# joybio/multiPrime

Measured on AMD Instinct MI355X. Metric: candidate x sequence coverage evals/s, higher is better.
Workload: dtype u32; 1 GPU; synthetic MSA 1048576 x 1000, k=18, v=1, 8 candidates/window, 950 windows, strict -c 2,3,-1 per GPU x 1 GPU(s) = BASELINE configs[3] itself (SURVEY 8d input 4; synthetic 1M x 1 kb; shape 1x1: row shards x window groups); rows_per_gpu=1048576, rows_total=1048576, cols=1000, k=18, variation=1, candidates_per_window=8, windows=950, parallelism=one GPU holds every row

## Files before the change

multiprime_amd/csrc/common.hpp:

```cpp
#pragma once

#include "../../include/mprime.h"

#include <hip/hip_runtime.h>

#include <algorithm>
#include <cstdarg>
#include <cstdio>
#include <cstdlib>
#include <cstring>
#include <numeric>
#include <utility>
#include <chrono>
#include <mutex>
#include <unordered_map>
#include <vector>

namespace mp {

constexpr int kBlock = 256;
constexpr uint32_t kEmpty = 0xFFFFFFFFu;
constexpr int kHashSlots = 4096;
constexpr int kHashLimit = 3584;
constexpr int kEvalCC = 8;
// ... 107 lines not shown
    hipStream_t ex_stream = nullptr;
    int ex_pending = 0;
    std::mutex ex_mu;
    int32_t *extra_off = nullptr;
    uint32_t *extra_words = nullptr;
    int n_extra = 0;
    std::vector<int32_t> h_patch_off, h_extra_off;
    uint32_t *pplanes = nullptr, *pvalid = nullptr;
    uint32_t *qplanes = nullptr, *qvalid = nullptr;
    bool qp_dirty = true;
    mp::PatchWin *pwin = nullptr;
    size_t pp_words = 0, pv_words = 0;
    int max_npw = 0;
    bool pp_dirty = true;
    unsigned long long *g_key = nullptr;
    uint32_t *g_cnt = nullptr, *g_min = nullptr;
    uint32_t *g_gap = nullptr;
    int32_t *g_idx = nullptr;
    int g_slots = 0;
    long long u_cap = 0, u_n = 0;
    uint32_t *u_b0 = nullptr, *u_b1 = nullptr, *u_g = nullptr;
    int32_t *u_count = nullptr, *u_first = nullptr, *labels = nullptr, *u_over = nullptr, *u_wcount = nullptr;
    int64_t *u_wbase = nullptr;
    unsigned long long *u_total = nullptr;
    std::vector<int64_t> h_wbase;
    std::vector<int32_t> h_wcount;
    double gate_threshold = 0;
    std::vector<uint8_t> h_wskip;
    uint8_t *dm_loss = nullptr;
    double *dm_dg = nullptr;
    std::vector<uint8_t> dm_loss_host;
    std::vector<double> dm_dg_host;
    unsigned long long *mask_f = nullptr, *mask_r = nullptr;
    size_t mask_words = 0;
    int n_masks = 0;
    int n_cand = 0, n_items = 0, n_padded = 0;
    mp::EvalItem *items = nullptr;
    uint4 *cand_n = nullptr;
    uint32_t *cand_symT = nullptr, *cand_diff = nullptr, *chain_events = nullptr;
    mp::ChainItem *chain_items = nullptr;
    void *x_items = nullptr;
    uint32_t *x_events = nullptr;
    int32_t *x_cand_out = nullptr;
    int x_n = 0, x_n_events = 0;
    int32_t *table_ids = nullptr;
    int n_chain = 0, n_table = 0, n_events = 0, max_steps = 0;
    std::vector<mp::ChainItem> h_chains;
    std::vector<uint32_t> h_events;
    std::vector<int32_t> h_cand_out;
    uint32_t *chain_prog = nullptr;
    size_t chain_prog_n = 0;
    mp::EvalForm form;
    mp::SlideBand *slide_bands = nullptr;
    uint32_t *slide_iters = nullptr, *slide_recs = nullptr;
    size_t slide_n_iters = 0;
    int slide_items = 0, slide_n_bands = 0, slide_max_items = 0, slide_ns = 0, slide_gw = 0;
    uint32_t slide_spos = 0, slide_fmask = 0, slide_rmask = 0, slide_fpos = 0, slide_rpos = 0;
    bool slide_fast = false;
    mp::ChainItem *chain_rest = nullptr;
    mp::ChainItem *chain_slid = nullptr;
    int n_rest = 0, rest_max_steps = 0;
    unsigned launch_seq = 0;
    int32_t *cand_out = nullptr;
    uint64_t sF = 0, sR = 0;
    unsigned long long *tmp_out = nullptr;
    int tmp_out_n = 0;
    struct PoolBlock { void *p; size_t bytes; hipEvent_t released; };
    std::vector<hipEvent_t> pool_events;
    std::unordered_map<void *, size_t> pool_live;
    std::vector<PoolBlock> pool;
    size_t pool_bytes = 0;
    long long pool_hits = 0, pool_misses = 0;
    int pool_on = -1;
    std::mutex pool_mu;
    unsigned long long *stats_buf = nullptr;
    size_t stats_buf_n = 0;
    std::vector<std::pair<hipEvent_t, hipEvent_t>> ev_busy, ev_free;
    double ev_ms = 0;
    std::vector<float> ev_samples, ev_last;
    int ev_n = 0;
    uint8_t *h_stage = nullptr;
    size_t h_stage_bytes = 0;
    bool h_stage_pinned = false;
    uint8_t *h_stats = nullptr;
    size_t h_stats_bytes = 0, stats_pending_f = 0, stats_pending_t = 0;
    bool h_stats_pinned = false;
    hipEvent_t stats_ev = nullptr;
    uint8_t *h_ring = nullptr;
    bool h_ring_pinned = false;
    hipEvent_t h_ring_ev[3] = {nullptr, nullptr, nullptr};
    uint8_t *sq_bytes = nullptr;
    int64_t *sq_roff = nullptr;
    unsigned long long *sq_code = nullptr, *sq_flag = nullptr;
    int64_t *sq_woff = nullptr;
    int32_t sq_n = 0;
    size_t sq_total = 0, sq_words = 0;
    std::vector<int64_t> sq_roff_host;
    int32_t *ot_out = nullptr;
    int64_t ot_n = 0;
    std::vector<uint8_t> ot_key;
    double ot_ms[4] = {0, 0, 0, 0};
    int64_t ot_counts[7] = {0, 0, 0, 0, 0, 0, 0};
    uint8_t *an_code = nullptr;
    uint32_t *an_kmer = nullptr;
    int32_t *an_table = nullptr;
    int32_t *an_col = nullptr, *an_colinv = nullptr;
    int32_t an_n = 0, an_L = 0, an_slots = 0;
// ... 122 lines not shown
```

multiprime_amd/csrc/evalslide.hip:

```cpp
#include "common.hpp"
#include "bitslice.hpp"
#include "slidecore.hpp"
#include "evalslide.hpp"
#include "chainbody.hpp"

using namespace mp;

namespace {

typedef unsigned int u32x4 __attribute__((ext_vector_type(4)));
typedef unsigned int u32x2 __attribute__((ext_vector_type(2)));

struct SlideKernArgs {
    SlideArgs A;
    const uint32_t *cols32;
    const uint32_t *excl32;
    int nw32;
    unsigned long long *out;
    int wc, wc_pad;
    int max_items;
    int n_slide_blocks;
    EvalChainArgs chain;
    unsigned long long *clear;
    uint32_t n_clear;
    int patch_words;
    unsigned long long *stamps;
};

template <int GW>
struct DevEnv {
    const SlideKernArgs &K;
    __amdgpu_buffer_rsrc_t rs_cols, rs_excl;
    int voff, lane;
    uint32_t row_bytes;
    bool live;
    uint32_t *ring;
    uint32_t *tab;
    uint32_t itv;
    uint32_t live_mask;

    __device__ __forceinline__ DevEnv(const SlideKernArgs &k) : K(k) {}
    __device__ __forceinline__ void progress(int quarter) const {
#ifndef SLIDE_NO_PRIO
        if (quarter <= 0) __builtin_amdgcn_s_setprio(3);
        else if (quarter == 1) __builtin_amdgcn_s_setprio(2);
        else if (quarter == 2) __builtin_amdgcn_s_setprio(1);
        else __builtin_amdgcn_s_setprio(0);
#endif
    }
    __device__ __forceinline__ void stamp(int i) const {
        if (K.stamps && threadIdx.x == 0) K.stamps[(size_t)blockIdx.x * 8 + i] = wall_clock64();
    }
    __device__ __forceinline__ SlideBand uband(int b) const {
        const SlideBand *p = K.A.bands + b;
        SlideBand r;
        r.w0 = __builtin_amdgcn_readfirstlane(p->w0); r.n_win = __builtin_amdgcn_readfirstlane(p->n_win);
        r.item0 = __builtin_amdgcn_readfirstlane(p->item0); r.n_items = __builtin_amdgcn_readfirstlane(p->n_items);
        r.iter0 = __builtin_amdgcn_readfirstlane(p->iter0); r.pad = 0;
        return r;
    }
    __device__ __forceinline__ void load_iters(int idx) { itv = K.A.iters[(size_t)idx + (size_t)lane]; }
    __device__ __forceinline__ uint32_t iter_word(int j) const { return (uint32_t)__builtin_amdgcn_readlane((int)itv, j); }
    typedef const uint32_t __attribute__((address_space(4))) * ConstWords;
    struct Rec { uint32_t w[8], sm_lo, sm_hi, flags; ConstWords p; };
    __device__ __forceinline__ Rec load_rec(int item) const {
        Rec r;
        r.p = (ConstWords)(K.A.recs + (size_t)__builtin_amdgcn_readfirstlane(item) * kSlideRec);
#pragma unroll
        for (int q = 0; q < 8; q++) r.w[q] = r.p[q];
        r.sm_lo = r.p[24]; r.sm_hi = r.p[25]; r.flags = r.p[28];
        return r;
    }
    __device__ __forceinline__ uint32_t rec_word(const Rec &r, int q) const {
        return q < 8 ? r.w[q] : (q == 24 ? r.sm_lo : (q == 25 ? r.sm_hi : (q == 28 ? r.flags : r.p[q])));
    }
    __device__ __forceinline__ uint32_t rec_word_dyn(const Rec &r, int q) const { return r.p[q]; }
    template <int AUX = 0>
    __device__ __forceinline__ void load(__amdgpu_buffer_rsrc_t rs, int soff, uint32_t (&d)[GW]) const {
        if constexpr (GW == 4) {
            const u32x4 v = __builtin_amdgcn_raw_buffer_load_b128(rs, voff, soff, AUX);
            d[0] = v.x; d[1] = v.y; d[2] = v.z; d[3] = v.w;
        } else if constexpr (GW == 2) {
            const u32x2 v = __builtin_amdgcn_raw_buffer_load_b64(rs, voff, soff, AUX);
            d[0] = v.x; d[1] = v.y;
        } else {
            d[0] = __builtin_amdgcn_raw_buffer_load_b32(rs, voff, soff, AUX);
        }
    }
#ifndef SLIDE_EXP_ONE_ROW
#define SLIDE_EXP_ONE_ROW 0
#endif
#ifndef SLIDE_COL_AUX
#define SLIDE_COL_AUX 2
#endif
#ifndef SLIDE_EVT_AUX
#define SLIDE_EVT_AUX 0
#endif
    __device__ __forceinline__ void fetch(uint32_t row_off, uint32_t (&d)[GW]) const {
        load<SLIDE_COL_AUX>(rs_cols, SLIDE_EXP_ONE_ROW == 1 || SLIDE_EXP_ONE_ROW == 3 ? 0 : (int)row_off, d);
    }
    __device__ __forceinline__ void fetch_event(uint32_t row_off, uint32_t (&d)[GW]) const {
// ... 46 lines not shown
            "v_add_u32_dpp %8, %8, %8 row_ror:8 row_mask:0xf bank_mask:0x3\n\t"
            "v_add_u32_dpp %0, %2, %2 row_ror:8 row_mask:0xf bank_mask:0xc\n\t"
            "v_add_u32_dpp %4, %6, %6 row_ror:8 row_mask:0xf bank_mask:0xc\n\t"
            "v_add_u32_dpp %8, %10, %10 row_ror:8 row_mask:0xf bank_mask:0xc\n\t"
            "v_add_u32_dpp %0, %0, %0 quad_perm:[1,0,3,2] row_mask:0xf bank_mask:0xf\n\t"
            "v_add_u32_dpp %4, %4, %4 quad_perm:[1,0,3,2] row_mask:0xf bank_mask:0xf\n\t"
            "v_add_u32_dpp %8, %8, %8 quad_perm:[1,0,3,2] row_mask:0xf bank_mask:0xf\n\t"
            "v_add_u32_dpp %0, %0, %0 quad_perm:[2,3,0,1] row_mask:0xf bank_mask:0xf\n\t"
            "v_add_u32_dpp %4, %4, %4 quad_perm:[2,3,0,1] row_mask:0xf bank_mask:0xf\n\t"
            "v_add_u32_dpp %8, %8, %8 quad_perm:[2,3,0,1] row_mask:0xf bank_mask:0xf\n\t"
            "s_nop 1"
            : "+v"(x0), "+v"(x1), "+v"(x2), "+v"(x3), "+v"(x4), "+v"(x5), "+v"(x6), "+v"(x7), "+v"(x8), "+v"(x9), "+v"(x10), "+v"(x11));
        typedef unsigned int u32pair __attribute__((ext_vector_type(2)));
        const u32pair s01 = __builtin_amdgcn_permlane16_swap(x0, x4, false, false);
        const uint32_t a = s01.x + s01.y;
        const u32pair s22 = __builtin_amdgcn_permlane16_swap(x8, x8, false, false);
        const uint32_t b = s22.x + s22.y;
        const u32pair h = __builtin_amdgcn_permlane32_swap(a, b, false, false);
        const uint32_t tot = h.x + h.y;
        if (lane < 48 && (lane & 3) == 0) atomicAdd(&tab[idx * 12 + (lane >> 4) * 4 + ((lane >> 2) & 3)], tot);
    }
};

#ifndef SLIDE_MIN_WAVES
#define SLIDE_MIN_WAVES 1
#endif
template <int LV, int GW, bool FAST>
__global__ __launch_bounds__(kBlock, GW == 4 ? 1 : SLIDE_MIN_WAVES) void eval_slide_kernel(const SlideKernArgs K) {
    extern __shared__ __align__(16) uint32_t lds[];
    clear_counters(K.clear, K.n_clear, blockIdx.x, gridDim.x);
    if (K.stamps && threadIdx.x == 0) K.stamps[(size_t)blockIdx.x * 8] = wall_clock64();
    if ((int)blockIdx.x >= K.n_slide_blocks) {
        const unsigned pb = blockIdx.x - (unsigned)K.n_slide_blocks, wv = threadIdx.x >> 6;
#ifndef SLIDE_PATCH_PRIO
#define SLIDE_PATCH_PRIO 3
#endif
        __builtin_amdgcn_s_setprio(SLIDE_PATCH_PRIO);
        if (K.patch_words == 1) {
            const bool negative = (int)pb >= K.chain.patch.n_blocks;
            const unsigned unit = (pb - (negative ? (unsigned)K.chain.patch.n_blocks : 0u)) * (kBlock / 64) + wv;
            eval_patch_wave<LV>(K.chain, lds + wv * 12, lds + 64 + wv * (64 * kPatchEvents), unit, negative);
        } else {
            uint32_t(&s_part)[kBlock / 64][12] = *reinterpret_cast<uint32_t(*)[kBlock / 64][12]>(lds);
            eval_chain_block<LV, 8, 4>(K.chain, s_part, pb);
        }
        if (K.stamps && threadIdx.x == 0) K.stamps[(size_t)blockIdx.x * 8 + 7] = wall_clock64();
        return;
    }
    const int slice = (int)(blockIdx.x % (unsigned)K.wc_pad), band = (int)(blockIdx.x / (unsigned)K.wc_pad);
    if (slice >= K.wc) return;
    const int wv = (int)(threadIdx.x >> 6), lane = (int)(threadIdx.x & 63);
    const int ring_words = K.A.k * 64 * GW;
    uint32_t *tab = lds + (kBlock / 64) * ring_words;
    DevEnv<GW> env(K);
    env.lane = lane;
    env.ring = lds + wv * ring_words + lane * GW;
    env.tab = tab;
    env.itv = 0u;
    const int word0 = (slice * kBlock + (int)threadIdx.x) * GW;
    env.live = word0 < K.nw32;
    env.voff = env.live ? word0 * 4 : 0x7FFFFF00;
    env.live_mask = env.live ? 0xFFFFFFFFu : 0u;
    env.row_bytes = (uint32_t)K.nw32 * 4u;
    env.rs_cols = __builtin_amdgcn_make_buffer_rsrc(const_cast<uint32_t *>(K.cols32), 0, 0x7FFFFF00, 0x00020000);
    env.rs_excl = __builtin_amdgcn_make_buffer_rsrc(const_cast<uint32_t *>(K.excl32), 0, 0x7FFFFF00, 0x00020000);
    const SlideBand bd = env.uband(band);
    for (int i = (int)threadIdx.x; i < bd.n_items * 12; i += kBlock) tab[i] = 0u;
    __syncthreads();
    env.stamp(1);
    const bool wave_live = (slice * kBlock + wv * 64) * GW < K.nw32;
    if (wave_live) slide_band<LV, GW, true, false, FAST>(env, K.A, band);
    env.stamp(4);
    __syncthreads();
    env.stamp(5);
    int live_waves = 0;
    for (int w = 0; w < kBlock / 64; w++) live_waves += (slice * kBlock + w * 64) * GW < K.nw32 ? 1 : 0;
    const uint32_t rows = (uint32_t)live_waves * 64u * 32u * GW;
    const int n_entries = bd.n_items * 24;
    for (int i0 = (int)threadIdx.x; i0 < n_entries; i0 += 4 * kBlock) {
        int oc[4];
        uint32_t map[4];
#pragma unroll
        for (int u = 0; u < 4; u++) {
            const int i = i0 + u * kBlock, ic = i < n_entries ? i : (int)threadIdx.x;
            const uint32_t *rec = K.A.recs + (size_t)(bd.item0 + ic / 24) * kSlideRec;
            oc[u] = (int)rec[8 + (ic % 24) / 3];
            map[u] = rec[26];
        }
#pragma unroll
        for (int u = 0; u < 4; u++) {
            const int i = i0 + u * kBlock;
            if (i >= n_entries || oc[u] < 0) continue;
            const int item = i / 24, r = i % 24, t = r / 3, kind = r % 3;
            const int slot = (int)((map[u] >> (4 * t)) & 15u);
            const uint32_t *row = tab + item * 12;
            const uint32_t out1 = row[slot] & 0xFFFFu, outF = row[slot] >> 16, outR = (row[8 + (slot >> 1)] >> (16 * (slot & 1))) & 0xFFFFu;
            const uint32_t val = kind == 0 ? rows - out1 : out1 - (kind == 1 ? outF : outR);
            if (val) atomicAdd(&K.out[(size_t)oc[u] * 3 + kind], (unsigned long long)val);
        }
    }
    env.stamp(6);
}

typedef void (*SlideFn)(const SlideKernArgs);

}

namespace mp {

void free_slide(mp_ctx *c) {
    dev_free(c, &c->slide_bands, (size_t)c->slide_n_bands);
    dev_free(c, &c->slide_iters, c->slide_n_iters);
    dev_free(c, &c->slide_recs, (size_t)c->slide_items * kSlideRec);
    dev_free(c, &c->chain_rest, (size_t)c->n_rest);
    dev_free(c, &c->chain_slid, (size_t)c->slide_items);
    c->slide_items = c->slide_n_bands = c->slide_max_items = 0;
    c->slide_n_iters = 0;
    c->n_rest = c->rest_max_steps = 0;
}

int upload_eval_slide(mp_ctx *c, const std::vector<ChainItem> &chains, const std::vector<uint32_t> &events, const std::vector<int32_t> &cand_out) {
    free_slide(c);
    const char *se = getenv("MP_EVAL_SLIDE");
    if (chains.empty() || c->v > 3 || c->k <= c->v || (se ? atoi(se) != 1 : c->n_pad <= 262144)) return MP_OK;
    const int nw32 = c->n_pad / 32, n_cols = c->n_chunks * 32;
    if (((unsigned long long)n_cols * 4ull + 1ull) * (unsigned long long)nw32 * 4ull >= 0x7FFFFFFFull) return MP_OK;
    if ((unsigned long long)c->n_win * (unsigned long long)nw32 * 4ull >= 0x7FFFFFFFull) return MP_OK;
    int gw = 2;
    if (const char *e = getenv("MP_SLIDE_GW")) { const int g = atoi(e); if (g == 1 || g == 2 || g == 4) gw = g; }
    const int wc = (nw32 + kBlock * gw - 1) / (kBlock * gw), wc_pad = wc >= 8 ? (wc + 7) / 8 * 8 : wc;
    const int span = chains.back().win - chains.front().win + 1;
    std::vector<SlideChainIn> in(chains.size());
    for (size_t i = 0; i < chains.size(); i++) {
        const ChainItem &ch = chains[i];
        in[i] = SlideChainIn{ch.win, ch.cand0, ch.n_steps, ch.ev0, ch.n_ev, {ch.sym[0], ch.sym[1], ch.sym[2], ch.sym[3]}};
    }
    const size_t ring_bytes = (size_t)(kBlock / 64) * ((size_t)c->k * 64 * gw) * sizeof(uint32_t), lds_cu = 160 * 1024;
    int resident = (int)std::min<size_t>(4, std::max<size_t>(1, lds_cu / (ring_bytes + 1024)));
    if (gw == 4) resident = 1;
    SlidePlan P;
    for (;; resident--) {
        const int per_round = std::max(1, 256 * resident / std::max(1, wc_pad));
        int band = (span + per_round - 1) / per_round;
        for (int r = 2; band > 96; r++) band = (span + per_round * r - 1) / (per_round * r);
        band = std::max(8, band);
        if (const char *e = getenv("MP_SLIDE_BAND")) band = std::max(1, atoi(e));
        if (!build_slide_plan(in, events, cand_out, c->k, (uint32_t)c->sF, (uint32_t)c->sR, c->p0, n_cols, band, (uint32_t)nw32 * 4u, true, P)) return MP_OK;
        const size_t need = ring_bytes + (size_t)P.max_items_band * 12 * sizeof(uint32_t);
        if (resident <= 1 || need * (size_t)resident <= lds_cu) break;
    }
    P.iters.resize(P.iters.size() + 64, 0u);
    int rc;
    if ((rc = dev_alloc(c, &c->slide_bands, P.bands.size()))) return rc;
    c->slide_n_bands = (int)P.bands.size();
    if ((rc = dev_alloc(c, &c->slide_iters, P.iters.size()))) return rc;
    c->slide_n_iters = P.iters.size();
    c->slide_items = (int)P.item_of.size();
    if ((rc = dev_alloc(c, &c->slide_recs, P.recs.size()))) return rc;
    HIPCK(c, hipMemcpy(c->slide_bands, P.bands.data(), sizeof(SlideBand) * P.bands.size(), hipMemcpyHostToDevice));
    HIPCK(c, hipMemcpy(c->slide_iters, P.iters.data(), sizeof(uint32_t) * P.iters.size(), hipMemcpyHostToDevice));
    HIPCK(c, hipMemcpy(c->slide_recs, P.recs.data(), sizeof(uint32_t) * P.recs.size(), hipMemcpyHostToDevice));
    c->slide_max_items = P.max_items_band;
    c->slide_ns = P.ns; c->slide_spos = P.spos; c->slide_fmask = P.fmask; c->slide_rmask = P.rmask;
    c->slide_fast = slide_strict_lists(c->k, (uint32_t)c->sF, (uint32_t)c->sR, c->slide_fpos, c->slide_rpos);
    if (const char *e = getenv("MP_SLIDE_STRICT")) { if (atoi(e) == 0) c->slide_fast = false; }
    c->slide_gw = gw;
    {
        std::vector<ChainItem> slid;
        for (int32_t i : P.item_of) slid.push_back(chains[(size_t)i]);
        if ((rc = dev_alloc(c, &c->chain_slid, slid.size()))) return rc;
        HIPCK(c, hipMemcpy(c->chain_slid, slid.data(), sizeof(ChainItem) * slid.size(), hipMemcpyHostToDevice));
    }
    if (!P.rest.empty()) {
        std::vector<ChainItem> rest;
        for (int32_t i : P.rest) { rest.push_back(chains[(size_t)i]); c->rest_max_steps = std::max(c->rest_max_steps, (int)chains[(size_t)i].n_steps); }
        if ((rc = dev_alloc(c, &c->chain_rest, rest.size()))) return rc;
        c->n_rest = (int)rest.size();
        HIPCK(c, hipMemcpy(c->chain_rest, rest.data(), sizeof(ChainItem) * rest.size(), hipMemcpyHostToDevice));
    }
    return MP_OK;
}

int launch_eval_slide(mp_ctx *c, unsigned long long *device_out, const EvalChainArgs *patch, int patch_blocks, int patch_words,
                      unsigned long long *clear, uint32_t n_clear) {
#define SLIDE_ROW(LV, F) {eval_slide_kernel<LV, 1, F>, eval_slide_kernel<LV, 2, F>, eval_slide_kernel<LV, 4, F>}
    static const SlideFn fn[2][4][3] = {{SLIDE_ROW(1, false), SLIDE_ROW(2, false), SLIDE_ROW(3, false), SLIDE_ROW(4, false)},
                                        {SLIDE_ROW(1, true), SLIDE_ROW(2, true), SLIDE_ROW(3, true), SLIDE_ROW(4, true)}};
#undef SLIDE_ROW
    const int gw = c->slide_gw, gi = gw == 4 ? 2 : gw - 1;
    const int nw32 = c->n_pad / 32;
    SlideKernArgs K;
    K.A = SlideArgs{c->slide_bands, c->slide_iters, c->slide_recs, c->k, c->p0, c->slide_ns, c->slide_spos, c->slide_fmask, c->slide_rmask,
                    (uint32_t)nw32 * 4u, c->slide_fpos, c->slide_rpos, 0u, 0u};
    if (c->slide_fast) slide_strict_distinct(c->slide_fpos, c->slide_rpos, K.A.dpos, K.A.dshape);
    K.cols32 = reinterpret_cast<const uint32_t *>(c->cols);
    K.excl32 = reinterpret_cast<const uint32_t *>(c->excl);
    K.nw32 = nw32;
    K.out = device_out;
    K.wc = (nw32 + kBlock * gw - 1) / (kBlock * gw);
    K.wc_pad = K.wc >= 8 ? (K.wc + 7) / 8 * 8 : K.wc;
    K.max_items = c->slide_max_items;
    K.n_slide_blocks = c->slide_n_bands * K.wc_pad;
    if (patch) K.chain = *patch;
    else { memset(&K.chain, 0, sizeof K.chain); patch_blocks = 0; }
    K.chain.clear = nullptr; K.chain.n_clear = 0;
    K.clear = clear; K.n_clear = n_clear;
    K.patch_words = patch_words;
    K.stamps = nullptr;
    const char *stamp_file = getenv("MP_EXPERIMENT_STAMPS");
    const size_t n_stamp = ((size_t)K.n_slide_blocks + (size_t)patch_blocks) * 8;
    if (stamp_file) {
        HIPCK(c, hipMalloc(&K.stamps, n_stamp * sizeof(unsigned long long)));
        HIPCK(c, hipMemsetAsync(K.stamps, 0, n_stamp * sizeof(unsigned long long), c->stream));
    }
    size_t lds = ((size_t)(kBlock / 64) * ((size_t)c->k * 64 * gw) + (size_t)c->slide_max_items * 12) * sizeof(uint32_t);
    if (patch_blocks) lds = std::max(lds, (size_t)(64 + (kBlock / 64) * 64 * kPatchEvents) * sizeof(uint32_t));
    if (lds > 160 * 1024) return fail(c, MP_ERR_ARG, "sliding evaluation: a band needs %zu bytes of LDS", lds);
    SlideFn f = fn[c->slide_fast ? 1 : 0][c->v][gi];
    if (lds > 48 * 1024) HIPCK(c, hipFuncSetAttribute(reinterpret_cast<const void *>(f), hipFuncAttributeMaxDynamicSharedMemorySize, (int)lds));
    hipLaunchKernelGGL(f, dim3((unsigned)K.n_slide_blocks + (unsigned)patch_blocks), dim3(kBlock), lds, c->stream, K);
    HIPCK(c, hipGetLastError());
    if (stamp_file) {
        std::vector<unsigned long long> h(n_stamp + 2);
        HIPCK(c, hipStreamSynchronize(c->stream));
        HIPCK(c, hipMemcpy(h.data() + 2, K.stamps, n_stamp * sizeof(unsigned long long), hipMemcpyDeviceToHost));
        HIPCK(c, hipFree(K.stamps));
        h[0] = (unsigned long long)K.n_slide_blocks; h[1] = (unsigned long long)patch_blocks;
        if (FILE *fo = fopen(stamp_file, "wb")) { fwrite(h.data(), sizeof(unsigned long long), h.size(), fo); fclose(fo); }
    }
    return MP_OK;
}

}
```

multiprime_amd/csrc/slidecore.hpp:

```cpp
#pragma once

#include <cstdint>

#include "slideplan.hpp"

#if defined(__HIPCC__)
#define SLIDE_HD __host__ __device__ __forceinline__
#else
#define SLIDE_HD inline
#endif

#ifndef SLIDE_UNLIKELY
#define SLIDE_UNLIKELY(x) __builtin_expect(!!(x), 0)
#endif

namespace mp {

template <int LUT>
SLIDE_HD uint32_t bop(uint32_t a, uint32_t b, uint32_t c) {
#if defined(__HIP_DEVICE_COMPILE__)
    return __builtin_amdgcn_bitop3_b32(a, b, c, LUT);
#else
    uint32_t r = 0;
    if (LUT & 0x01) r |= ~a & ~b & ~c;
    if (LUT & 0x02) r |= ~a & ~b & c;
    if (LUT & 0x04) r |= ~a & b & ~c;
    if (LUT & 0x08) r |= ~a & b & c;
    if (LUT & 0x10) r |= a & ~b & ~c;
    if (LUT & 0x20) r |= a & ~b & c;
    if (LUT & 0x40) r |= a & b & ~c;
    if (LUT & 0x80) r |= a & b & c;
    return r;
#endif
}
constexpr int slide_lut(bool (*f)(bool, bool, bool)) {
    int t = 0;
    for (int i = 0; i < 8; i++)
        if (f((i >> 2) & 1, (i >> 1) & 1, i & 1)) t |= 1 << i;
    return t;
}
constexpr int kSlXor3 = slide_lut([](bool a, bool b, bool c) { return (a != b) != c; });
constexpr int kSlMaj = slide_lut([](bool a, bool b, bool c) { return (a && b) || (a && c) || (b && c); });
constexpr int kSlProp = slide_lut([](bool p, bool ci, bool dir) { return p && (ci == dir); });
constexpr int kSlBorrow = slide_lut([](bool ci, bool s, bool br) { return (!ci && s) || (!ci && br) || (s && br); });
constexpr int kSlAndNot = slide_lut([](bool a, bool b, bool) { return a && !b; });
constexpr int kSlOr3 = slide_lut([](bool a, bool b, bool c) { return a || b || c; });
constexpr int kSlOrAnd = slide_lut([](bool a, bool b, bool c) { return a || (b && c); });
constexpr int kSlOrAndNot = slide_lut([](bool a, bool b, bool c) { return a || (b && !c); });
constexpr int kSlAndNotNot = slide_lut([](bool a, bool b, bool c) { return a && !b && !c; });
constexpr int kSlOrNot = slide_lut([](bool a, bool b, bool) { return a || !b; });
constexpr int kSlOrOrNot = slide_lut([](bool a, bool b, bool c) { return a || b || !c; });
constexpr int kSlXorAndNot = slide_lut([](bool a, bool b, bool c) { return a != (b && !c); });

SLIDE_HD int slide_popc(uint32_t x) {
#if defined(__HIP_DEVICE_COMPILE__)
    return __popc(x);
#else
    return __builtin_popcount(x);
#endif
}

SLIDE_HD void slide_pin(uint32_t &x) {
#if defined(__HIP_DEVICE_COMPILE__)
    asm volatile("" : "+v"(x));
#else
    (void)x;
#endif
}

struct SlideCount { uint32_t b0, b1, b2, b3, b4; };
SLIDE_HD void slide_updown(SlideCount &c, uint32_t x, uint32_t dir) {
    uint32_t p = x;
    uint32_t n = c.b0 ^ p; p = bop<kSlProp>(p, c.b0, dir); c.b0 = n;
    n = c.b1 ^ p; p = bop<kSlProp>(p, c.b1, dir); c.b1 = n;
    n = c.b2 ^ p; p = bop<kSlProp>(p, c.b2, dir); c.b2 = n;
    n = c.b3 ^ p; p = bop<kSlProp>(p, c.b3, dir); c.b3 = n;
    c.b4 ^= p;
}

struct SlideArgs {
    const SlideBand *bands;
    const uint32_t *iters;
    const uint32_t *recs;
    int k, p0, ns;
    uint32_t spos, fmask, rmask;
    uint32_t row_scale;
    uint32_t fpos, rpos;
    uint32_t dpos, dshape;
};

inline bool slide_strict_lists(int k, uint32_t sF, uint32_t sR, uint32_t &fpos, uint32_t &rpos) {
    fpos = rpos = 0u;
    uint32_t nf = 0, nr = 0;
    for (int j = 0; j < k && j < 32; j++) {
        if ((sF >> j) & 1u) { if (nf == 3) return false; fpos |= (uint32_t)j << (5 * nf++); }
        if ((sR >> j) & 1u) { if (nr == 3) return false; rpos |= (uint32_t)j << (5 * nr++); }
    }
    fpos |= nf << 15; rpos |= nr << 15;
    return true;
}

inline void slide_strict_distinct(uint32_t fpos, uint32_t rpos, uint32_t &dpos, uint32_t &dshape) {
    const int nf = (int)(fpos >> 15), nr = (int)(rpos >> 15);
    uint32_t fm = 0, rm = 0;
    for (int q = 0; q < nf; q++) fm |= 1u << ((fpos >> (5 * q)) & 31u);
    for (int q = 0; q < nr; q++) rm |= 1u << ((rpos >> (5 * q)) & 31u);
    const uint32_t sets[3] = {fm & rm, fm & ~rm, rm & ~fm};
    int n = 0, cnt[3] = {0, 0, 0};
    dpos = 0u;
    for (int c = 0; c < 3; c++)
        for (int j = 0; j < 32; j++)
            if ((sets[c] >> j) & 1u) { dpos |= (uint32_t)j << (5 * n++); cnt[c]++; }
    dshape = (uint32_t)cnt[0] | ((uint32_t)cnt[1] << 2) | ((uint32_t)cnt[2] << 4);
}
constexpr uint32_t slide_shape_code(int nb, int nfo, int nro) { return (uint32_t)nb | ((uint32_t)nfo << 2) | ((uint32_t)nro << 4); }
constexpr uint32_t kSlShapeDefault = slide_shape_code(1, 1, 2);

template <int NB_, int NFO_, int NRO_, bool MASKED_>
struct SlideShape { static constexpr int NB = NB_, NFO = NFO_, NRO = NRO_, ND = NB_ + NFO_ + NRO_; static constexpr bool MASKED = MASKED_; };

template <int GW>
struct SlideFetch {
    uint32_t d[kSlideKept + 1][GW];
    uint32_t valid[GW];
};

template <int GW, bool USE_VALID, class Env>
SLIDE_HD void slide_request(Env &env, const typename Env::Rec &rec, SlideFetch<GW> &F) {
    if (USE_VALID) env.valid_of(env.rec_word(rec, 29), F.valid);
#pragma unroll
    for (int s = 1; s <= kSlideKept; s++) env.fetch_event(env.rec_word(rec, s), F.d[s]);
}

template <int LV, int GW, bool SIMPLE, bool USE_VALID, bool NO_EXTRA, bool FAST, class Env>
SLIDE_HD void slide_item(Env &env, const SlideArgs &A, const typename Env::Rec &rec, uint32_t hdr, const SlideCount (&cnt)[GW],
                         const uint32_t (&sv)[kSlideStrict][GW], const SlideFetch<GW> &F, uint32_t (&accPF)[8], uint32_t (&accR)[4]) {
    const int n_extra = (int)((hdr >> 8) & 15u);
    const uint32_t flags = env.rec_word(rec, 28);
    SlideCount c0[GW];
    uint32_t sub[kSlideKept + 1];
#pragma unroll
// ... 180 lines not shown
        cur += env.ring_step();
    }
}

template <int LV, int GW, bool ONLY_SIMPLE, bool USE_VALID, bool FAST = false, class Env>
SLIDE_HD void slide_band(Env &env, const SlideArgs &A, int band_index) {
    static_assert(LV >= 1 && LV <= 4 && GW >= 1 && GW <= 4, "counter levels / words per lane");
    static_assert(!FAST || ONLY_SIMPLE, "FAST strict counts: simple items only");
    const SlideBand bd = env.uband(band_index);
    const int k = A.k;
    SlideCount cnt[GW];
#pragma unroll
    for (int i = 0; i < GW; i++) cnt[i] = SlideCount{0u, 0u, 0u, 0u, 0u};
    env.ring_zero(k);
    const uint32_t ring_step = env.ring_step(), ring_end = (uint32_t)k * ring_step;
    uint32_t cur = 0u;
    const int n_iter = bd.n_win + k - 1;
    const int last_item = bd.item0 + bd.n_items - 1;
    typename Env::Rec rec0 = env.load_rec(bd.item0), rec1 = env.load_rec(bd.item0 + 1 <= last_item ? bd.item0 + 1 : last_item);
    SlideFetch<GW> F0, F1;
    slide_request<GW, USE_VALID>(env, rec0, F0);
    int done = 0;
    env.load_iters(bd.iter0);
    env.stamp(2);
    int j0 = 0;
    {
        const int n_warm = k - 1 < n_iter ? k - 1 : n_iter;
        while (n_warm - j0 >= 16) { slide_warm_chunk<16, GW>(env, cnt, cur, j0); j0 += 16; }
        if (n_warm - j0 >= 8) { slide_warm_chunk<8, GW>(env, cnt, cur, j0); j0 += 8; }
        if (n_warm - j0 >= 4) { slide_warm_chunk<4, GW>(env, cnt, cur, j0); j0 += 4; }
        if (n_warm - j0 >= 2) { slide_warm_chunk<2, GW>(env, cnt, cur, j0); j0 += 2; }
    }
    env.stamp(3);
    uint32_t bA[GW], bB[GW];
    env.fetch(env.iter_word(2 * j0), bA);
    env.fetch(env.iter_word(n_iter > j0 + 1 ? 2 * j0 + 2 : 2 * j0), bB);

    auto item = [&](typename Env::Rec &rec_cur, typename Env::Rec &rec_other, const SlideFetch<GW> &F_cur, SlideFetch<GW> &F_other,
                    const uint32_t (&sv)[kSlideStrict][GW]) __attribute__((always_inline)) {
        const int after = bd.item0 + done + 2;
        const typename Env::Rec rec = rec_cur;
        rec_cur = env.load_rec(after <= last_item ? after : last_item);
        slide_request<GW, USE_VALID>(env, rec_other, F_other);
        const uint32_t hdr = env.rec_word(rec, 0);
        uint32_t accPF[8], accR[4];
        if (ONLY_SIMPLE || (hdr & kSlSimple)) slide_item<LV, GW, true, USE_VALID, ONLY_SIMPLE, FAST>(env, A, rec, hdr, cnt, sv, F_cur, accPF, accR);
        else slide_item<LV, GW, false, USE_VALID, false, false>(env, A, rec, hdr, cnt, sv, F_cur, accPF, accR);
        env.commit(done, accPF, accR);
        done++;
    };
#ifndef SLIDE_PRIO_MIN_WIN
#define SLIDE_PRIO_MIN_WIN 32
#endif
    const int quarter_len = bd.n_win < SLIDE_PRIO_MIN_WIN ? 1 << 20 : ((bd.n_win + 3) / 4 > 2 ? (bd.n_win + 3) / 4 : 2);
    auto run = [&](auto shape) __attribute__((always_inline)) {
        typedef decltype(shape) Shape;
        constexpr int NS = Shape::ND;
        uint32_t so[NS > 0 ? NS : 1], sm[NS > 0 ? NS : 1];
#pragma unroll
        for (int q = 0; q < NS; q++) {
            uint32_t pos, present = 1u;
            if (!FAST) pos = (A.spos >> (5 * q)) & 31u;
            else if (!Shape::MASKED) pos = (A.dpos >> (5 * q)) & 31u;
            else {
                const uint32_t list = q < 3 ? A.fpos : A.rpos;
                const int qq = q < 3 ? q : q - 3;
                present = qq < (int)(list >> 15) ? 1u : 0u;
                pos = present ? (list >> (5 * qq)) & 31u : 0u;
            }
            so[q] = (((uint32_t)j0 + pos) % (uint32_t)k) * ring_step;
            sm[q] = present ? 0xFFFFFFFFu : 0u;
        }
        auto iteration = [&](uint32_t (&b)[GW], uint32_t (&bo)[GW], uint32_t (&bo_next)[GW], int j) __attribute__((always_inline)) {
            const uint32_t it1 = env.iter_word(2 * j + 1);
            uint32_t bn[GW];
#pragma unroll
            for (int i = 0; i < GW; i++) bn[i] = ~b[i];
            env.fetch(env.iter_word(2 * j + 4), b);
#pragma unroll
            for (int i = 0; i < GW; i++) slide_updown(cnt[i], bn[i] ^ bo[i], bn[i]);
            env.ring_write(cur, bn);
            cur += ring_step;
            if (cur == ring_end) cur = 0u;
            env.ring_read(cur, bo_next);
#pragma unroll
            for (int q = 0; q < NS; q++) {
                so[q] += ring_step;
                if (so[q] == ring_end) so[q] = 0u;
            }
            const int n_items = (int)(it1 >> 24);
            if (n_items == 0) return;
            uint32_t sv[kSlideStrict][GW];
            if (FAST) {
                uint32_t d[NS > 0 ? NS : 1][GW];
#pragma unroll
                for (int q = 0; q < NS; q++) {
                    env.ring_read(so[q], d[q]);
                    if (Shape::MASKED) {
#pragma unroll
                        for (int i = 0; i < GW; i++) d[q][i] &= sm[q];
                    }
                }
                constexpr int NF = Shape::NB + Shape::NFO, NR = Shape::NB + Shape::NRO;
                static_assert(NF <= 3 && NR <= 3, "at most three strict positions per side");
#pragma unroll
                for (int i = 0; i < GW; i++) {
                    uint32_t f[3] = {0u, 0u, 0u}, r[3] = {0u, 0u, 0u};
#pragma unroll
                    for (int q = 0; q < NF; q++) f[q] = d[q][i];
#pragma unroll
                    for (int q = 0; q < NR; q++) r[q] = d[q < Shape::NB ? q : q + Shape::NFO][i];
                    sv[0][i] = NF == 3 ? bop<kSlXor3>(f[0], f[1], f[2]) : (f[0] ^ f[1]);
                    sv[1][i] = NF == 3 ? bop<kSlMaj>(f[0], f[1], f[2]) : (f[0] & f[1]);
                    sv[2][i] = NR == 3 ? bop<kSlXor3>(r[0], r[1], r[2]) : (r[0] ^ r[1]);
                    sv[3][i] = NR == 3 ? bop<kSlMaj>(r[0], r[1], r[2]) : (r[0] & r[1]);
                }
            }
#pragma unroll
            for (int q = 0; q < kSlideStrict; q++) {
                if (FAST) break;
                if (q < NS) {
                    env.ring_read(so[q], sv[q]);
                } else {
#pragma unroll
                    for (int i = 0; i < GW; i++) sv[q][i] = 0u;
                }
            }
            int ii = 0;
            if (done & 1) { item(rec1, rec0, F1, F0, sv); ii = 1; }
#pragma unroll 1
            for (; ii + 1 < n_items; ii += 2) {
                item(rec0, rec1, F0, F1, sv);
                item(rec1, rec0, F1, F0, sv);
            }
            if (ii < n_items) item(rec0, rec1, F0, F1, sv);
        };
        int quarter = 0, next_quarter = k - 1 + quarter_len;
        env.progress(0);
        uint32_t boA[GW], boB[GW];
        env.ring_read(cur, boA);
#pragma unroll 1
        for (int base = 0; base < n_iter; base += 30) {
            if (base) env.load_iters(bd.iter0 + 2 * base);
            const int n_here = n_iter - base < 30 ? n_iter - base : 30;
            int j = base ? 0 : j0;
#pragma unroll 1
            for (; j + 1 < n_here; j += 2) {
                if (base + j >= next_quarter) { env.progress(++quarter); next_quarter += quarter_len; }
                iteration(bA, boA, boB, j);
                iteration(bB, boB, boA, j + 1);
            }
            if (j < n_here) iteration(bA, boA, boB, j);
        }
    };
    if constexpr (!FAST) {
        if (A.ns > 4) run(SlideShape<0, 3, 3, false>());
        else run(SlideShape<0, 2, 2, false>());
    } else {
        switch (A.dshape) {
            case kSlShapeDefault: run(SlideShape<1, 1, 2, false>()); break;
            case slide_shape_code(0, 0, 0): run(SlideShape<0, 0, 0, false>()); break;
            case slide_shape_code(1, 0, 0): run(SlideShape<1, 0, 0, false>()); break;
            case slide_shape_code(0, 1, 1): run(SlideShape<0, 1, 1, false>()); break;
            case slide_shape_code(0, 2, 2): run(SlideShape<0, 2, 2, false>()); break;
            case slide_shape_code(0, 3, 3): run(SlideShape<0, 3, 3, false>()); break;
            default: run(SlideShape<0, 3, 3, true>()); break;
        }
    }
    env.progress(3);
}

}
```

multiprime_amd/csrc/slideplan.hpp:

```cpp
#pragma once

#include <algorithm>
#include <cstdint>
#include <cstring>
#include <vector>

namespace mp {

constexpr int kSlideRec = 32;
constexpr int kSlideKept = 7;
constexpr int kSlideExtra = 8;
constexpr int kSlideStrict = 6;
constexpr uint32_t kSlPresent = 1u << 7, kSlSub = 1u << 8, kSlStrictF = 1u << 9, kSlStrictR = 1u << 10;
constexpr uint32_t kSlSimple = 1u << 16;

struct SlideChainIn {
    int32_t win, cand0, n_steps, ev0, n_ev;
    uint32_t sym[4];
};

struct SlideBand { int32_t w0, n_win, item0, n_items, iter0, pad; };

struct SlidePlan {
    std::vector<uint8_t> slides;
    std::vector<int32_t> rest;
    std::vector<int32_t> item_of;
    std::vector<SlideBand> bands;
    std::vector<uint32_t> iters;
    std::vector<uint32_t> recs;
    std::vector<uint8_t> ref;
    int k = 0, ns = 0, max_items_band = 0;
    uint32_t spos = 0, fmask = 0, rmask = 0;
};

inline bool slide_record(const SlideChainIn &ch, const std::vector<uint32_t> &events, const std::vector<int32_t> &cand_out, int k, uint32_t sF,
                         uint32_t sR, int p0, const std::vector<uint8_t> &ref, const int (&slot_of_pos)[32], uint32_t row_scale,
                         uint32_t zero_row, uint32_t *rec) {
    auto sym = [&](int j) { return (ch.sym[j >> 3] >> (4 * (j & 7))) & 15u; };
    for (int q = 0; q < kSlideRec; q++) rec[q] = 0u;
    if (ch.n_steps < 1 || ch.n_steps > 8) return false;
    for (int m = 0; m < 8; m++) rec[8 + m] = 0xFFFFFFFFu;
    for (int q = 1; q <= kSlideKept; q++) rec[q] = zero_row * row_scale;
    const uint32_t row0 = (uint32_t)(p0 + ch.win) * 4u;
    int cur = 0, e = 0;
    rec[8] = (uint32_t)cand_out[(size_t)ch.cand0];
    bool lost_seen[32 * 4] = {false};
    bool simple = true;
    for (int t = 1; t < ch.n_steps; t++) {
        while (e < ch.n_ev && (int)(events[(size_t)ch.ev0 + (size_t)e] >> 16) == t) {
            const uint32_t ev = events[(size_t)ch.ev0 + (size_t)e];
            const int j = (int)(ev & 255u), base = __builtin_ctz((ev >> 8) & 15u);
            if (++cur > kSlideKept) return false;
            rec[cur] = (row0 + (uint32_t)(j * 4 + base)) * row_scale;
            if ((sF >> j) & 1u) rec[28] |= 1u << cur;
            if ((sR >> j) & 1u) rec[28] |= 1u << (8 + cur);
            if (base != ref[(size_t)(p0 + ch.win + j)]) {
                rec[28] |= 1u << (16 + cur);
                if (slot_of_pos[j] >= 0) rec[24 + slot_of_pos[j] / 4] |= (1u << cur) << (8 * (slot_of_pos[j] & 3));
            } else {
                simple = false;
            }
            lost_seen[j * 4 + base] = true;
            e++;
        }
        rec[8 + t] = (uint32_t)cand_out[(size_t)ch.cand0 + (size_t)t];
        rec[26] |= (uint32_t)cur << (4 * t);
    }
    if (e != ch.n_ev) return false;
    int nx = 0;
    for (int j = 0; j < k; j++) {
        const uint32_t sy = sym(j);
        const int r = ref[(size_t)(p0 + ch.win + j)];
        for (int b = 0; b < 4; b++) {
            const bool in_s0 = sy >> b & 1u;
            const bool sub = in_s0 && b != r && !lost_seen[j * 4 + b], add = !in_s0 && b == r;
            if (!sub && !add) continue;
            if (slot_of_pos[j] >= 0 || nx == kSlideExtra) return false;
            rec[16 + nx++] = (uint32_t)(j * 4 + b) | kSlPresent | (sub ? kSlSub : 0u);
        }
    }
    rec[0] = (uint32_t)(cur + 1) | ((uint32_t)nx << 8) | (simple ? kSlSimple : 0u);
    rec[27] = (uint32_t)ch.win;
    rec[29] = (uint32_t)ch.win * row_scale;
    rec[30] = row0 * row_scale;
    return true;
}

inline bool build_slide_plan(const std::vector<SlideChainIn> &chains, const std::vector<uint32_t> &events, const std::vector<int32_t> &cand_out,
                             int k, uint32_t sF, uint32_t sR, int p0, int n_cols, int band_windows, uint32_t row_scale, bool simple_only,
                             SlidePlan &P) {
    P = SlidePlan();
    P.k = k;
    if (k < 2 || k > 31 || chains.empty()) return false;
    const uint32_t kmask = (1u << k) - 1u;
    int slot_of_pos[32];
    for (int j = 0; j < 32; j++) slot_of_pos[j] = -1;
    for (int j = 0; j < k; j++)
        if (((sF | sR) & kmask) >> j & 1u) {
            if (P.ns == kSlideStrict) return false;
            slot_of_pos[j] = P.ns;
            P.spos |= (uint32_t)j << (5 * P.ns);
            if ((sF >> j) & 1u) P.fmask |= 1u << P.ns;
            if ((sR >> j) & 1u) P.rmask |= 1u << P.ns;
            P.ns++;
        }
    auto sym = [](const SlideChainIn &ch, int j) { return (ch.sym[j >> 3] >> (4 * (j & 7))) & 15u; };
    std::vector<int32_t> votes((size_t)n_cols * 4, 0);
    for (const SlideChainIn &ch : chains) {
        if (ch.win < 0 || p0 + ch.win + k > n_cols) return false;
        for (int j = 0; j < k; j++)
            for (int b = 0; b < 4; b++)
                if (sym(ch, j) >> b & 1u) votes[(size_t)(p0 + ch.win + j) * 4 + b]++;
    }
    P.ref.assign((size_t)n_cols, 0);
    for (int c = 0; c < n_cols; c++) {
        int best = 0;
        for (int b = 1; b < 4; b++)
            if (votes[(size_t)c * 4 + b] > votes[(size_t)c * 4 + best]) best = b;
        P.ref[(size_t)c] = (uint8_t)best;
    }
    P.slides.assign(chains.size(), 0);
    std::vector<uint32_t> rec((size_t)kSlideRec);
    for (size_t i = 0; i < chains.size(); i++) {
        if (i && chains[i].win < chains[i - 1].win) return false;
        if (slide_record(chains[i], events, cand_out, k, sF, sR, p0, P.ref, slot_of_pos, row_scale, (uint32_t)n_cols * 4u, rec.data()) &&
            (!simple_only || ((rec[0] & kSlSimple) && ((rec[0] >> 8) & 15u) == 0))) {
            P.slides[i] = 1;
            P.item_of.push_back((int32_t)i);
            P.recs.insert(P.recs.end(), rec.begin(), rec.end());
        } else {
            P.rest.push_back((int32_t)i);
        }
    }
    if (P.item_of.empty()) return false;
    const int B = std::max(1, band_windows);
    const size_t n = P.item_of.size();
    auto win_of = [&](size_t pi) { return chains[(size_t)P.item_of[pi]].win; };
    size_t i = 0;
    while (i < n) {
        SlideBand bd{win_of(i), 1, (int32_t)i, 0, (int32_t)P.iters.size(), 0};
        size_t j = i;
        int last = win_of(i);
        while (j < n) {
            const int w = win_of(j);
            if (w - bd.w0 + 1 > B || w - last > k - 1) break;
            last = w;
            j++;
        }
        bd.n_win = last - bd.w0 + 1;
        bd.n_items = (int32_t)(j - i);
        P.max_items_band = std::max(P.max_items_band, (int)bd.n_items);
        size_t it = i;
        for (int t = -(k - 1); t < bd.n_win; t++) {
            const int col = p0 + bd.w0 + t + k - 1;
            uint32_t first = (uint32_t)(it - i), cnt = 0;
            if (t >= 0)
                while (it < j && win_of(it) == bd.w0 + t) { it++; cnt++; }
            if (cnt > 255) return false;
            P.iters.push_back(((uint32_t)col * 4u + P.ref[(size_t)col]) * row_scale);
            P.iters.push_back(first | (cnt << 24));
        }
        P.bands.push_back(bd);
        i = j;
    }
    return true;
}

}
```

Before: 63960 billion evals/s.

## Precompute packed flush words and optionally flush counts in-band per quarter

```diff
diff --git a/multiprime_amd/csrc/common.hpp b/multiprime_amd/csrc/common.hpp
--- a/multiprime_amd/csrc/common.hpp
+++ b/multiprime_amd/csrc/common.hpp
@@ -183,7 +183,7 @@
     size_t chain_prog_n = 0;
     mp::EvalForm form;
     mp::SlideBand *slide_bands = nullptr;
-    uint32_t *slide_iters = nullptr, *slide_recs = nullptr;
+    uint32_t *slide_iters = nullptr, *slide_recs = nullptr, *slide_flush = nullptr;
     size_t slide_n_iters = 0;
     int slide_items = 0, slide_n_bands = 0, slide_max_items = 0, slide_ns = 0, slide_gw = 0;
     uint32_t slide_spos = 0, slide_fmask = 0, slide_rmask = 0, slide_fpos = 0, slide_rpos = 0;
diff --git a/multiprime_amd/csrc/evalslide.hip b/multiprime_amd/csrc/evalslide.hip
--- a/multiprime_amd/csrc/evalslide.hip
+++ b/multiprime_amd/csrc/evalslide.hip
@@ -27,6 +27,10 @@
     unsigned long long *stamps;
 };
 
+#ifndef SLIDE_FLUSH_UNROLL
+#define SLIDE_FLUSH_UNROLL 2
+#endif
+
 template <int GW>
 struct DevEnv {
     const SlideKernArgs &K;
@@ -38,6 +42,10 @@
     uint32_t *tab;
     uint32_t itv;
     uint32_t live_mask;
+    uint32_t *arrive;
+    const uint32_t *flush;
+    int live_waves;
+    uint32_t rows;
 
     __device__ __forceinline__ DevEnv(const SlideKernArgs &k) : K(k) {}
     __device__ __forceinline__ void progress(int quarter) const {
@@ -47,6 +55,35 @@
         else if (quarter == 2) __builtin_amdgcn_s_setprio(1);
         else __builtin_amdgcn_s_setprio(0);
 #endif
+    }
+    __device__ __forceinline__ void flush_entry(int i, uint32_t word) const {
+        if (word == kSlideNoFlush) return;
+        const int item = i / kSlideFlushEntries, kind = i % 3;
+        const int slot = (int)(word >> kSlideFlushCandBits);
+        const uint32_t *row = tab + item * 12;
+        const uint32_t out1 = row[slot] & 0xFFFFu, outF = row[slot] >> 16, outR = (row[8 + (slot >> 1)] >> (16 * (slot & 1))) & 0xFFFFu;
+        const uint32_t val = kind == 0 ? rows - out1 : out1 - (kind == 1 ? outF : outR);
+        if (val) atomicAdd(&K.out[(size_t)(word & ((1u << kSlideFlushCandBits) - 1u)) * 3 + kind], (unsigned long long)val);
+    }
+    template <int STRIDE, int U>
+    __device__ __forceinline__ void flush_entries(int first, int end) const {
+#pragma unroll 1
+        for (int i0 = first; i0 < end; i0 += U * STRIDE) {
+            uint32_t word[U];
+#pragma unroll
+            for (int u = 0; u < U; u++) word[u] = i0 + u * STRIDE < end ? flush[i0 + u * STRIDE] : kSlideNoFlush;
+#pragma unroll
+            for (int u = 0; u < U; u++) flush_entry(i0 + u * STRIDE, word[u]);
+        }
+    }
+    static constexpr uint32_t kArrived = 0x80000000u;
+    __device__ __forceinline__ void quarter_done(int q, int item_begin, int item_end) const {
+        if (item_begin == item_end) return;
+        uint32_t before = 0u;
+        if (lane == 0) before = __hip_atomic_fetch_add(&arrive[q], 1u, __ATOMIC_ACQ_REL, __HIP_MEMORY_SCOPE_WORKGROUP);
+        if ((int)__builtin_amdgcn_readfirstlane(before) != live_waves - 1) return;
+        flush_entries<64, SLIDE_FLUSH_UNROLL>(item_begin * kSlideFlushEntries + lane, item_end * kSlideFlushEntries);
+        if (lane == 0) arrive[q] = kArrived | (uint32_t)item_end;
     }
     __device__ __forceinline__ void stamp(int i) const {
         if (K.stamps && threadIdx.x == 0) K.stamps[(size_t)blockIdx.x * 8 + i] = wall_clock64();
@@ -199,6 +236,7 @@
     const int wv = (int)(threadIdx.x >> 6), lane = (int)(threadIdx.x & 63);
     const int ring_words = K.A.k * 64 * GW;
     uint32_t *tab = lds + (kBlock / 64) * ring_words;
+    uint32_t *arrive = tab + K.max_items * 12;
     DevEnv<GW> env(K);
     env.lane = lane;
     env.ring = lds + wv * ring_words + lane * GW;
@@ -213,6 +251,13 @@
     env.rs_excl = __builtin_amdgcn_make_buffer_rsrc(const_cast<uint32_t *>(K.excl32), 0, 0x7FFFFF00, 0x00020000);
     const SlideBand bd = env.uband(band);
     for (int i = (int)threadIdx.x; i < bd.n_items * 12; i += kBlock) tab[i] = 0u;
+    if (threadIdx.x < SLIDE_FLUSH_POINTS) arrive[threadIdx.x] = 0u;
+    int live_waves = 0;
+    for (int w = 0; w < kBlock / 64; w++) live_waves += (slice * kBlock + w * 64) * GW < K.nw32 ? 1 : 0;
+    env.arrive = arrive;
+    env.flush = K.A.flush + (size_t)bd.item0 * kSlideFlushEntries;
+    env.live_waves = live_waves;
+    env.rows = (uint32_t)live_waves * 64u * 32u * GW;
     __syncthreads();
     env.stamp(1);
     const bool wave_live = (slice * kBlock + wv * 64) * GW < K.nw32;
@@ -220,32 +265,15 @@
     env.stamp(4);
     __syncthreads();
     env.stamp(5);
-    int live_waves = 0;
-    for (int w = 0; w < kBlock / 64; w++) live_waves += (slice * kBlock + w * 64) * GW < K.nw32 ? 1 : 0;
-    const uint32_t rows = (uint32_t)live_waves * 64u * 32u * GW;
-    const int n_entries = bd.n_items * 24;
-    for (int i0 = (int)threadIdx.x; i0 < n_entries; i0 += 4 * kBlock) {
-        int oc[4];
-        uint32_t map[4];
-#pragma unroll
-        for (int u = 0; u < 4; u++) {
-            const int i = i0 + u * kBlock, ic = i < n_entries ? i : (int)threadIdx.x;
-            const uint32_t *rec = K.A.recs + (size_t)(bd.item0 + ic / 24) * kSlideRec;
-            oc[u] = (int)rec[8 + (ic % 24) / 3];
-            map[u] = rec[26];
-        }
-#pragma unroll
-        for (int u = 0; u < 4; u++) {
-            const int i = i0 + u * kBlock;
-            if (i >= n_entries || oc[u] < 0) continue;
-            const int item = i / 24, r = i % 24, t = r / 3, kind = r % 3;
-            const int slot = (int)((map[u] >> (4 * t)) & 15u);
-            const uint32_t *row = tab + item * 12;
-            const uint32_t out1 = row[slot] & 0xFFFFu, outF = row[slot] >> 16, outR = (row[8 + (slot >> 1)] >> (16 * (slot & 1))) & 0xFFFFu;
-            const uint32_t val = kind == 0 ? rows - out1 : out1 - (kind == 1 ? outF : outR);
-            if (val) atomicAdd(&K.out[(size_t)oc[u] * 3 + kind], (unsigned long long)val);
-        }
-    }
+    int from = 0;
+#if SLIDE_FLUSH_INBAND
+#pragma unroll
+    for (int q = 0; q < SLIDE_FLUSH_POINTS; q++) {
+        const uint32_t a = arrive[q];
+        if ((a & DevEnv<GW>::kArrived) && (int)(a & ~DevEnv<GW>::kArrived) > from) from = (int)(a & ~DevEnv<GW>::kArrived);
+    }
+#endif
+    env.template flush_entries<kBlock, 4>(from * kSlideFlushEntries + (int)threadIdx.x, bd.n_items * kSlideFlushEntries);
     env.stamp(6);
 }
 
@@ -259,6 +287,7 @@
     dev_free(c, &c->slide_bands, (size_t)c->slide_n_bands);
     dev_free(c, &c->slide_iters, c->slide_n_iters);
     dev_free(c, &c->slide_recs, (size_t)c->slide_items * kSlideRec);
+    dev_free(c, &c->slide_flush, (size_t)c->slide_items * kSlideFlushEntries);
     dev_free(c, &c->chain_rest, (size_t)c->n_rest);
     dev_free(c, &c->chain_slid, (size_t)c->slide_items);
     c->slide_items = c->slide_n_bands = c->slide_max_items = 0;
@@ -293,7 +322,7 @@
         band = std::max(8, band);
         if (const char *e = getenv("MP_SLIDE_BAND")) band = std::max(1, atoi(e));
         if (!build_slide_plan(in, events, cand_out, c->k, (uint32_t)c->sF, (uint32_t)c->sR, c->p0, n_cols, band, (uint32_t)nw32 * 4u, true, P)) return MP_OK;
-        const size_t need = ring_bytes + (size_t)P.max_items_band * 12 * sizeof(uint32_t);
+        const size_t need = ring_bytes + ((size_t)P.max_items_band * 12 + SLIDE_FLUSH_POINTS) * sizeof(uint32_t);
         if (resident <= 1 || need * (size_t)resident <= lds_cu) break;
     }
     P.iters.resize(P.iters.size() + 64, 0u);
@@ -307,6 +336,8 @@
     HIPCK(c, hipMemcpy(c->slide_bands, P.bands.data(), sizeof(SlideBand) * P.bands.size(), hipMemcpyHostToDevice));
     HIPCK(c, hipMemcpy(c->slide_iters, P.iters.data(), sizeof(uint32_t) * P.iters.size(), hipMemcpyHostToDevice));
     HIPCK(c, hipMemcpy(c->slide_recs, P.recs.data(), sizeof(uint32_t) * P.recs.size(), hipMemcpyHostToDevice));
+    if ((rc = dev_alloc(c, &c->slide_flush, P.flush.size()))) return rc;
+    HIPCK(c, hipMemcpy(c->slide_flush, P.flush.data(), sizeof(uint32_t) * P.flush.size(), hipMemcpyHostToDevice));
     c->slide_max_items = P.max_items_band;
     c->slide_ns = P.ns; c->slide_spos = P.spos; c->slide_fmask = P.fmask; c->slide_rmask = P.rmask;
     c->slide_fast = slide_strict_lists(c->k, (uint32_t)c->sF, (uint32_t)c->sR, c->slide_fpos, c->slide_rpos);
@@ -338,7 +369,7 @@
     const int nw32 = c->n_pad / 32;
     SlideKernArgs K;
     K.A = SlideArgs{c->slide_bands, c->slide_iters, c->slide_recs, c->k, c->p0, c->slide_ns, c->slide_spos, c->slide_fmask, c->slide_rmask,
-                    (uint32_t)nw32 * 4u, c->slide_fpos, c->slide_rpos, 0u, 0u};
+                    (uint32_t)nw32 * 4u, c->slide_fpos, c->slide_rpos, 0u, 0u, c->slide_flush};
     if (c->slide_fast) slide_strict_distinct(c->slide_fpos, c->slide_rpos, K.A.dpos, K.A.dshape);
     K.cols32 = reinterpret_cast<const uint32_t *>(c->cols);
     K.excl32 = reinterpret_cast<const uint32_t *>(c->excl);
@@ -360,7 +391,7 @@
         HIPCK(c, hipMalloc(&K.stamps, n_stamp * sizeof(unsigned long long)));
         HIPCK(c, hipMemsetAsync(K.stamps, 0, n_stamp * sizeof(unsigned long long), c->stream));
     }
-    size_t lds = ((size_t)(kBlock / 64) * ((size_t)c->k * 64 * gw) + (size_t)c->slide_max_items * 12) * sizeof(uint32_t);
+    size_t lds = ((size_t)(kBlock / 64) * ((size_t)c->k * 64 * gw) + (size_t)c->slide_max_items * 12 + SLIDE_FLUSH_POINTS) * sizeof(uint32_t);
     if (patch_blocks) lds = std::max(lds, (size_t)(64 + (kBlock / 64) * 64 * kPatchEvents) * sizeof(uint32_t));
     if (lds > 160 * 1024) return fail(c, MP_ERR_ARG, "sliding evaluation: a band needs %zu bytes of LDS", lds);
     SlideFn f = fn[c->slide_fast ? 1 : 0][c->v][gi];
diff --git a/multiprime_amd/csrc/slidecore.hpp b/multiprime_amd/csrc/slidecore.hpp
--- a/multiprime_amd/csrc/slidecore.hpp
+++ b/multiprime_amd/csrc/slidecore.hpp
@@ -12,6 +12,13 @@
 
 #ifndef SLIDE_UNLIKELY
 #define SLIDE_UNLIKELY(x) __builtin_expect(!!(x), 0)
+#endif
+
+#ifndef SLIDE_FLUSH_INBAND
+#define SLIDE_FLUSH_INBAND 0
+#endif
+#ifndef SLIDE_FLUSH_POINTS
+#define SLIDE_FLUSH_POINTS 4
 #endif
 
 namespace mp {
@@ -87,6 +94,7 @@
     uint32_t row_scale;
     uint32_t fpos, rpos;
     uint32_t dpos, dshape;
+    const uint32_t *flush;
 };
 
 inline bool slide_strict_lists(int k, uint32_t sF, uint32_t sR, uint32_t &fpos, uint32_t &rpos) {
@@ -373,7 +381,9 @@
 #ifndef SLIDE_PRIO_MIN_WIN
 #define SLIDE_PRIO_MIN_WIN 32
 #endif
-    const int quarter_len = bd.n_win < SLIDE_PRIO_MIN_WIN ? 1 << 20 : ((bd.n_win + 3) / 4 > 2 ? (bd.n_win + 3) / 4 : 2);
+    static_assert(SLIDE_FLUSH_POINTS >= 4 && SLIDE_FLUSH_POINTS % 4 == 0, "flush points: quarters of the band or finer");
+    constexpr int kParts = SLIDE_FLUSH_POINTS;
+    const int quarter_len = bd.n_win < SLIDE_PRIO_MIN_WIN ? 1 << 20 : ((bd.n_win + kParts - 1) / kParts > 2 ? (bd.n_win + kParts - 1) / kParts : 2);
     auto run = [&](auto shape) __attribute__((always_inline)) {
         typedef decltype(shape) Shape;
         constexpr int NS = Shape::ND;
@@ -456,7 +466,7 @@
             }
             if (ii < n_items) item(rec0, rec1, F0, F1, sv);
         };
-        int quarter = 0, next_quarter = k - 1 + quarter_len;
+        int quarter = 0, next_quarter = k - 1 + quarter_len, flushed = 0;
         env.progress(0);
         uint32_t boA[GW], boB[GW];
         env.ring_read(cur, boA);
@@ -467,7 +477,11 @@
             int j = base ? 0 : j0;
 #pragma unroll 1
             for (; j + 1 < n_here; j += 2) {
-                if (base + j >= next_quarter) { env.progress(++quarter); next_quarter += quarter_len; }
+                if (base + j >= next_quarter) {
+                    env.progress(++quarter * 4 / kParts);
+                    next_quarter += quarter_len;
+                    if (SLIDE_FLUSH_INBAND) { env.quarter_done(quarter - 1, flushed, done); flushed = done; }
+                }
                 iteration(bA, boA, boB, j);
                 iteration(bB, boB, boA, j + 1);
             }
diff --git a/multiprime_amd/csrc/slideplan.hpp b/multiprime_amd/csrc/slideplan.hpp
--- a/multiprime_amd/csrc/slideplan.hpp
+++ b/multiprime_amd/csrc/slideplan.hpp
@@ -13,6 +13,9 @@
 constexpr int kSlideStrict = 6;
 constexpr uint32_t kSlPresent = 1u << 7, kSlSub = 1u << 8, kSlStrictF = 1u << 9, kSlStrictR = 1u << 10;
 constexpr uint32_t kSlSimple = 1u << 16;
+constexpr int kSlideFlushEntries = 24;
+constexpr int kSlideFlushCandBits = 28;
+constexpr uint32_t kSlideNoFlush = 0xFFFFFFFFu;
 
 struct SlideChainIn {
     int32_t win, cand0, n_steps, ev0, n_ev;
@@ -28,6 +31,7 @@
     std::vector<SlideBand> bands;
     std::vector<uint32_t> iters;
     std::vector<uint32_t> recs;
+    std::vector<uint32_t> flush;
     std::vector<uint8_t> ref;
     int k = 0, ns = 0, max_items_band = 0;
     uint32_t spos = 0, fmask = 0, rmask = 0;
@@ -86,6 +90,16 @@
     return true;
 }
 
+inline bool slide_flush_words(const uint32_t *rec, uint32_t *out) {
+    for (int t = 0; t < 8; t++) {
+        const int32_t oc = (int32_t)rec[8 + t];
+        if (oc >= (int32_t)(1u << kSlideFlushCandBits)) return false;
+        const uint32_t word = oc < 0 ? kSlideNoFlush : (uint32_t)oc | (((rec[26] >> (4 * t)) & 15u) << kSlideFlushCandBits);
+        for (int kind = 0; kind < 3; kind++) out[t * 3 + kind] = word;
+    }
+    return true;
+}
+
 inline bool build_slide_plan(const std::vector<SlideChainIn> &chains, const std::vector<uint32_t> &events, const std::vector<int32_t> &cand_out,
                              int k, uint32_t sF, uint32_t sR, int p0, int n_cols, int band_windows, uint32_t row_scale, bool simple_only,
                              SlidePlan &P) {
@@ -133,6 +147,9 @@
         }
     }
     if (P.item_of.empty()) return false;
+    P.flush.resize(P.item_of.size() * kSlideFlushEntries);
+    for (size_t pi = 0; pi < P.item_of.size(); pi++)
+        if (!slide_flush_words(P.recs.data() + pi * kSlideRec, P.flush.data() + pi * kSlideFlushEntries)) return false;
     const int B = std::max(1, band_windows);
     const size_t n = P.item_of.size();
     auto win_of = [&](size_t pi) { return chains[(size_t)P.item_of[pi]].win; };
```

Result: no change. 64590 billion evals/s, median of 6 (+1.0%).
